# Tycro-Games/Raytracer-VoxPopuli

Measured on AMD Instinct MI355X. Metric: Mray/s (primary+shadow) at 1920×1080, 1024³ world; 1/2/4/8-GPU, higher is better.
Workload: dtype f32

## Files before the change

### raytracer-voxpopuli_amd/csrc/vpx_kernels.hip

```cpp
#include <hip/hip_runtime.h>
#include <hip/hip_gl_interop.h>
#include <rccl/rccl.h>

#include <algorithm>
#include <cmath>
#include <cstdio>
#include <cstdlib>
#include <cstring>
#include <string>
#include <array>
#include <atomic>
#include <vector>

#include "vpx_wavefront.hpp"
#include "vpx_model.hpp"
#include "vpx_noise.hpp"
#include "vpx_brush.hpp"

using namespace vpx;

namespace {

constexpr int kTile = 16;
#ifndef VPX_SPLIT_PRIMARY
// ... 1249 lines not shown
        free_fork(ws);
        return fail(c, VPX_E_DEVICE, "level fork: stream / event creation failed");
    }
    return VPX_OK;
}
void free_fork(vpx_ctx::WaveStore& ws) {
    if (ws.fork) (void)hipStreamSynchronize(ws.fork);
    if (ws.ev_fork) (void)hipEventDestroy(ws.ev_fork);
    if (ws.ev_join) (void)hipEventDestroy(ws.ev_join);
    if (ws.fork) (void)hipStreamDestroy(ws.fork);
    if (ws.fork_dedicated) g_lane_queues.fetch_sub(1);
    ws.fork = nullptr, ws.ev_fork = ws.ev_join = nullptr, ws.fork_dedicated = false;
}

static void prof_mark(vpx_ctx* c, hipStream_t s, int stage) {
    if (!c->prof_cap) return;
    if (stage >= 0 && !((c->prof_mask >> stage) & 1u)) return;
    if (stage >= 0 && c->prof_used + 2 > c->prof_cap) return;
    if (stage < 0 && (c->prof_used & 1u) == 0) return;
    if (hipEventRecord(c->prof_ev[c->prof_used], s) != hipSuccess) return;
    c->prof_stage[c->prof_used] = stage;
    ++c->prof_used;
}

struct Reproj {
    PrevCam prev;
    float4 *alb, *ill, *rd, *temp, *hist;
};

template <int MODE>
int launch_render(vpx_ctx* c, hipStream_t s, vpx_ctx::WaveStore& ws, const SceneView& sv, const FrameArgs& f,
                  uint32_t tiles, float4* accum, uint32_t* rgb8, float4* packed, const Reproj* rp = nullptr,
                  const hipEvent_t* tail_wait = nullptr, const WindowTail* wtail = nullptr) {
    const uint32_t P = tiles * (uint32_t)kTilePix;
    const uint32_t L = (uint32_t)std::max(1, f.max_bounces + 1);
    const uint32_t S = sv.num_areas ? (uint32_t)std::max(1, sv.area_samples) : 1u;
    int rc = ensure_wave(c, ws, P, L, S);
    if (rc) return rc;
    WaveBufs w = ws.w;
    if (rp) w.RD = rp->rd;
    const dim3 grid(tiles), block(kThreads);
    const size_t slds = sizeof(uint32_t) * S * kThreads;
    const bool one = sv.num_volumes == 1 && !(sv.num_spheres | sv.num_triangles);
    const bool x86 = sv.x86.tab != nullptr;
    const size_t xlds = x86 ? sizeof(uint32_t) * sv.x86.rsq_off : 0;
    const bool fuse_tail = !rp;
#ifndef VPX_SPOOL_ONE_SLOT
#define VPX_SPOOL_ONE_SLOT 1
#endif
#ifndef VPX_SPOOL_ONE_SERIAL
#define VPX_SPOOL_ONE_SERIAL 0
#endif
    const bool spool = !rp && (S > 1 || (one && VPX_SPOOL_ONE_SLOT && (VPX_SPOOL_ONE_SERIAL || &ws != &c->wave)));
    if (wtail && (!spool || f.max_bounces < 0 || !f.batch_tiles || tiles % wtail->B))
        return fail(c, VPX_E_INVALID, "window tail: needs a window chain with the shadow pool");
    if (!spool) w.occb = nullptr;
    const uint32_t sgrab = std::max(1u, std::min(4u, kShadowList / (64u * S)));
    auto resident = [&](uint32_t waves_per_simd) { return dim3(std::min(tiles, c->cus * waves_per_simd)); };
    auto shadow_pool = [&](int level) {
        const uint32_t grabs = (P / 64u + sgrab - 1u) / sgrab;
        const uint32_t waves = std::min(grabs, c->cus * 4u * (uint32_t)VPX_WPE_SPOOL);
        const uint32_t wpb = kPoolWg / 64u;
        hipLaunchKernelGGL(one ? k_shadow_pool<false> : k_shadow_pool<true>, dim3((waves + wpb - 1u) / wpb), dim3(kPoolWg), 0,
                           s, sv, w, level, sgrab, c->d_ctr);
        if (!one)
            hipLaunchKernelGGL(k_shadow_slots, dim3(std::min(tiles * S, c->cus * (uint32_t)VPX_WPE_SHADOW_SLOTS)), block, 0, s, sv,
                               w, level, c->d_ctr);
    };
    c->last_frame_kernel = 0;
    if (frame0_fits(sv, f, S, rp != nullptr) && tiles <= kFuseFrameTiles) {
        prof_mark(c, s, VPX_STAGE_FRAME);
#ifndef VPX_FRAME_EXTRA_LDS
#define VPX_FRAME_EXTRA_LDS 0
#endif
#ifndef VPX_FRAME_VIEWS
#define VPX_FRAME_VIEWS 2
#endif
        constexpr int kBase = VPX_FRAME_VIEWS >= 1 ? kFrameGuaranteed : kFrameAsGiven;
        constexpr int kLean = VPX_FRAME_VIEWS >= 2 ? kFrameLean : kBase;
        const bool lean = VPX_FRAME_VIEWS >= 2 && frame0_lean(sv, f);
        c->last_frame_kernel = lean ? 2 : 1;
        hipLaunchKernelGGL((lean ? (x86 ? k_frame0<true, MODE, true, kLean> : k_frame0<true, MODE, false, kLean>)
                                 : (x86 ? k_frame0<true, MODE, true, kBase> : k_frame0<true, MODE, false, kBase>)),
                           grid, block, slds + VPX_FRAME_EXTRA_LDS, s, sv, f, w, c->d_ctr, accum, rgb8, packed);
        prof_mark(c, s, -1);
        VPX_HIP(c, hipGetLastError());
        return VPX_OK;
    }
    VPX_HIP(c, hipMemsetAsync(w.pool, 0, sizeof(uint32_t) * kPoolWords, s));
    prof_mark(c, s, VPX_STAGE_PRIMARY);
    const bool fuse_head = f.max_bounces >= 0;
    const bool split = !one && fuse_head && VPX_SPLIT_PRIMARY && !(sv.num_spheres | sv.num_triangles);
    const bool defer = split && f.max_bounces == 0 && VPX_DEFER_INSTANCES;
    if (defer)
        hipLaunchKernelGGL((x86 ? k_primary<true, true, true, true> : k_primary<true, true, false, true>), grid, block, 0, s,
                           sv, f, w, c->d_ctr);
    else if (split)
        hipLaunchKernelGGL((x86 ? k_primary<true, false, true> : k_primary<true, false, false>), grid, block, 0, s, sv, f, w,
                           c->d_ctr);
    else if (fuse_head)
        hipLaunchKernelGGL((one ? (x86 ? k_primary<true, true, true> : k_primary<true, true, false>)
                                : (x86 ? k_primary<false, true, true> : k_primary<false, true, false>)),
                           grid, block, 0, s, sv, f, w,
                           c->d_ctr);
    else
        hipLaunchKernelGGL((one ? (x86 ? k_primary<true, false, true> : k_primary<true, false, false>)
                                : (x86 ? k_primary<false, false, true> : k_primary<false, false, false>)),
                           grid, block, 0, s, sv, f,
                           w, c->d_ctr);
    prof_mark(c, s, -1);
    if (split) {
        prof_mark(c, s, VPX_STAGE_INSTANCES);
        if (defer) {
            hipLaunchKernelGGL(k_compact, dim3((P / 64u + 255u) / 256u), block, 0, s, w, 0);
            hipLaunchKernelGGL(k_instances_list, grid, block, xlds, s, sv, f, w, c->d_ctr);
        } else {
            hipLaunchKernelGGL(k_instances, grid, block, xlds, s, sv, f, w, c->d_ctr);
        }
        prof_mark(c, s, -1);
    }
    auto bounce = [&](hipStream_t bs, int level) {
        prof_mark(c, bs, VPX_STAGE_BOUNCE);
        if (one) {
            const uint32_t chunks = (P + kPoolChunk - 1u) / kPoolChunk;
            const uint32_t waves = std::min(chunks, c->cus * 4u * (uint32_t)VPX_WPE_BOUNCE);
            const uint32_t wpb = kPoolWg / 64u;
            hipLaunchKernelGGL(x86 ? k_nearest_pool<true> : k_nearest_pool<false>, dim3((waves + wpb - 1u) / wpb),
                               dim3(kPoolWg), 0, bs, sv, w, level,
                               c->d_ctr);
        } else {
            hipLaunchKernelGGL(k_nearest_tile, grid, block, xlds, bs, sv, w, level, c->d_ctr);
        }
        prof_mark(c, bs, -1);
    };
    const bool fork = VPX_LEVEL_FORK && f.max_bounces > 0 && !rp && (&ws == &c->wave || (one && c->lanes.size() <= 2));
    if (fork && (rc = ensure_fork(c, ws))) return rc;
    const int tail_at = &ws == &c->wave ? VPX_TAIL_LEVEL - 1 : VPX_TAIL_LEVEL;
    const int tail_from = (VPX_TAIL_LEVEL > 0 && f.max_bounces >= VPX_TAIL_MIN_DEPTH && !rp) ? tail_at : -1;
    bool tailed = false;
    for (int level = 0; level <= f.max_bounces; ++level) {
        if (!(fuse_head && level == 0)) {
            prof_mark(c, s, VPX_STAGE_SHADE);
            hipLaunchKernelGGL(k_shade, grid, block, 0, s, sv, f, w, level, c->d_ctr);
            prof_mark(c, s, -1);
        }
        if (fuse_tail && level == f.max_bounces) {
            prof_mark(c, s, VPX_STAGE_SHADOW);
            if (spool)
                shadow_pool(level);
            else
                hipLaunchKernelGGL((one ? k_shadow_finish<true, MODE> : k_shadow_finish<false, MODE>), grid, block,
                                   slds, s, sv, f, w, c->d_ctr, accum, rgb8, packed);
            prof_mark(c, s, -1);
            if (spool) {
                if (tail_wait) VPX_HIP(c, hipStreamWaitEvent(s, *tail_wait, 0));
                prof_mark(c, s, VPX_STAGE_FINISH);
                if (wtail)
                    hipLaunchKernelGGL(k_finish_window<true>, dim3(tiles / wtail->B), block, 0, s, sv, f, w, *wtail,
                                       accum, rgb8);
                else
                    hipLaunchKernelGGL((k_resolve_finish<MODE>), grid, block, 0, s, sv, f, w, accum, rgb8, packed);
                prof_mark(c, s, -1);
            }
            break;
        }
        if (level < f.max_bounces)
            hipLaunchKernelGGL(k_compact, dim3((P / 64u + 255u) / 256u), block, 0, s, w, level);
// ... 1948 lines not shown
```

### raytracer-voxpopuli_amd/csrc/vpx_wavefront.hpp

```cpp
#pragma once

#include "vpx_trace.hpp"

namespace vpx {

constexpr int kTileW = 16;
constexpr int kTilePix = kTileW * kTileW;



constexpr uint32_t kActive = 1u;
constexpr uint32_t kInside = 2u;

constexpr uint32_t kSlotValid = 1u;
constexpr uint32_t kSlotDiscard = 2u;

constexpr uint32_t kFlagReproject = 0x80000000u;
constexpr uint32_t kPendZeroAdd = 1u << 13;

constexpr uint32_t kLightNone = 0, kLightSingle = 1, kLightArea = 2;

struct FrameArgs {
    vpx_camera cam;
    uint32_t width, height;
// ... 628 lines not shown
        base += i < wid ? v : 0u;
        total += v;
    }
    __syncthreads();
    return base + off;
}

template <class KIND = NearestWalk>
__device__ __forceinline__ void nearest_record(SceneView sv, const PathRay& pr, uint32_t p, Ray& r, Counters& k) {
    r.t = kBig;
    r.mat = kNone;
    r.N = mk(0.f, 0.f, 0.f);
    const int32_t vox = find_nearest<KIND>(sv, r, k);
    pr.H[pr.at(p)] = make_float4(r.t, r.N.x, r.N.y, r.N.z);
    pr.HM[pr.at(p)] = r.mat | ((uint32_t)(vox + 2) << 8) | (r.inside ? 0x80000000u : 0u);
}

__device__ __forceinline__ ORay path_oray(const vpx_volume& vol, const PathRay& pr, uint32_t p,
                                          const X86Arith& xa = X86Arith{}) {
    const float4 o = pr.O[pr.at(p)], d = pr.D[pr.at(p)];
    ORay r;
    r.O = xform_pos_ssem(mk(o.x, o.y, o.z), vol.inv_matrix);
    r.D = xform_vec_ssem(mk(d.x, d.y, d.z), vol.inv_matrix);
    r.rD = nearest_rd(r.D, xa);
    return r;
}

__device__ __forceinline__ bool nearest_begin_v(const vpx_volume& vol, uint32_t n, const PathRay& w, uint32_t p,
                                                Counters& k, skip::Walk& wk, const X86Arith& xa) {
    ++k.nearest;
    const ORay o = path_oray(vol, w, p, xa);
    Dda s;
    if (!dda_setup(vol, n, o, s)) return false;
    wk = to_walk(s);
    return true;
}
__device__ __forceinline__ bool nearest_begin_1v(const SceneView& sv, const PathRay& w, uint32_t p, Counters& k,
                                                 skip::Walk& wk) {
    const vpx_volume* vol = uni_ptr(&sv.volumes[0]);
    return nearest_begin_v(*vol, sv.grids[vol->grid_id].n, w, p, k, wk, sv.x86);
}
__device__ __forceinline__ void nearest_end_v(const vpx_volume& vol, const uint8_t* cells, uint32_t n, const PathRay& w,
                                              uint32_t p, const skip::Walk& wk, bool hit);
__device__ __forceinline__ void nearest_end_1v(const SceneView& sv, const PathRay& w, uint32_t p, const skip::Walk& wk,
                                               bool hit) {
    const vpx_volume* vol = uni_ptr(&sv.volumes[0]);
    const DevGrid g = sv.grids[vol->grid_id];
    nearest_end_v(*vol, g.cells, g.n, w, p, wk, hit);
}

template <class KIND = NearestWalk>
__device__ __forceinline__ void nearest_record_1v(const SceneView& sv, const PathRay& w, uint32_t p, Counters& k) {
    bool hit = false;
    skip::Walk wk;
    if (nearest_begin_1v(sv, w, p, k, wk))
        hit = walk_wave<KIND>(grid_view(sv.grids[uni_ptr(&sv.volumes[0])->grid_id]), wk, kBig, k.cells);
    nearest_end_1v(sv, w, p, wk, hit);
}

__device__ __forceinline__ void nearest_end_v(const vpx_volume& vol, const uint8_t* cells, uint32_t n, const PathRay& w,
                                              uint32_t p, const skip::Walk& wk, bool hit) {
    asm volatile("" ::: "memory");
    const uint32_t inside = __float_as_uint(w.D[w.at(p)].w) & kInside ? 0x80000000u : 0u;
    if (!hit) {
        w.H[w.at(p)] = make_float4(kBig, 0.f, 0.f, 0.f);
        w.HM[w.at(p)] = kNone | inside;
        return;
    }
    const ORay o = path_oray(vol, w, p);
    const f3 N = normal_voxel(o, wk.t, n, vol.matrix);
    const uint32_t mat = cells[(uint64_t)wk.X + (uint64_t)wk.Y * n + (uint64_t)wk.Z * ((uint64_t)n * n)];
    w.H[w.at(p)] = make_float4(wk.t, N.x, N.y, N.z);
    w.HM[w.at(p)] = mat | (2u << 8) | inside;
}

template <bool SHADE>
struct HeadLds {
    uint32_t sh[4];
    uint32_t lst[256];
    float4 ray[SHADE ? 3 * 256 : 1];
    uint32_t hm[SHADE ? 256 : 1];
};

__device__ __forceinline__ bool meets_later_volume(const SceneView& sv, f3 o, f3 d, float t) {
    if (!(sv.tlas_on && !sv.tlas_always && !(sv.num_spheres | sv.num_triangles) && sv.tlas_nodes)) return true;
    return tlas_box(sv.tlas[0], o, world_inv(d), t);
}

template <bool ONE, bool SHADE, class KIND = NearestWalk, bool DEFER = false>
__device__ __forceinline__ void primary_tile(const SceneView& sv, const FrameArgs& f, const WaveBufs& w,
                                             HeadLds<SHADE>& L, unsigned long long* __restrict__ ctr) {
    uint32_t* sh = L.sh;
    uint32_t* lst = L.lst;
    const uint32_t tb = tile_block() * 256u;
    const uint32_t p = tb + threadIdx.x;
    const PathRay pr = SHADE ? PathRay{L.ray, L.ray + 256, L.ray + 512, L.hm, tb} : PathRay{w.O, w.D, w.H, w.HM, 0u};
    Counters k{0u, 0u, 0u};
    uint32_t prim = 0;
    bool walk = false;
    if (p < w.P) {
        uint32_t x, y;
        bool go = path_pixel(f, p, x, y);
        if (!SHADE) {
            w.depth[p] = f.max_bounces;
            w.forms[p] = 1u;
        }
        Ray r;
        r.O = r.D = mk(0.f, 0.f, 0.f);
        uint32_t rng = 0, flags = 0;
        if (go) {
            Rng g{pixel_seed(f.seed_base, path_frame(f, p), f.width, f.height, x, y)};
            r = primary_ray(f, x, y, g, sv.x86);
            rng = g.s;
            prim = 1;
            flags = kActive;
        }
        if (f.max_bounces < 0) {
            go = false;
            flags = 0u;
        }
        pr.O[pr.at(p)] = make_float4(r.O.x, r.O.y, r.O.z, __uint_as_float(rng));
        pr.D[pr.at(p)] = make_float4(r.D.x, r.D.y, r.D.z, __uint_as_float(flags));
        if (SHADE && !flags && f.max_bounces > 0) w.D[p] = make_float4(0.f, 0.f, 0.f, __uint_as_float(0u));
        if (go) {
            walk = true;
            if (ONE) {
                const vpx_volume& vol = sv.volumes[0];
                ORay o;
                o.O = xform_pos_ssem(r.O, vol.inv_matrix);
                o.D = xform_vec_ssem(r.D, vol.inv_matrix);
                o.rD = nearest_rd(o.D, sv.x86);
                Dda s;
                if (!dda_setup(vol, sv.grids[vol.grid_id].n, o, s)) {
                    walk = false;
                    ++k.nearest;
                    pr.H[pr.at(p)] = make_float4(kBig, 0.f, 0.f, 0.f);
                    pr.HM[pr.at(p)] = kNone;
                }
            }
        }
    }
    uint32_t total;
    const uint32_t at = block_scan(walk ? 1u : 0u, total, sh);
    if (walk) lst[at] = p;
    __syncthreads();
    VPX_FRAME_PHASE(1);
    if (threadIdx.x < total) {
        const uint32_t q = lst[threadIdx.x];
        if (ONE) {
            nearest_record_1v<KIND>(sv, pr, q, k);
        } else {
            const float4 o = pr.O[pr.at(q)], d = pr.D[pr.at(q)];
            Ray r;
            r.O = mk(o.x, o.y, o.z);
            r.D = mk(d.x, d.y, d.z);
            r.inside = false;
            nearest_record(sv, pr, q, r, k);
        }
    }
    VPX_FRAME_PHASE(2);
    flush_counters(k, prim, ctr, VPX_STAGE_PRIMARY);
    if (SHADE) {
        __syncthreads();
        VPX_FRAME_PHASE(3);
        Counters ks{0u, 0u, 0u};
        bool defer = false;
        if (DEFER && p < w.P) {
            const float4 d = pr.D[pr.at(p)];
            if (__float_as_uint(d.w) & kActive) {
                const float4 o = pr.O[pr.at(p)], h = pr.H[pr.at(p)];
                defer = meets_later_volume(sv, mk(o.x, o.y, o.z), mk(d.x, d.y, d.z), h.x);
                if (defer) {
                    w.O[p] = o;
                    w.D[p] = d;
                    w.H[p] = h;
                    w.HM[p] = pr.HM[pr.at(p)];
                }
            }
        }
        if (DEFER) put_amask(w, p, defer);
        const bool cont = defer ? false : shade_path<true>(sv, f, w, pr, p, 0, ks);
        if (!DEFER && f.max_bounces > 0) put_amask(w, p, cont);
        flush_counters(ks, 0u, ctr, VPX_STAGE_SHADE);
    }
}

template <bool ONE, bool SHADE = false, bool X86 = false, bool DEFER = false>
__global__ __launch_bounds__(256) VPX_WPE(ONE ? VPX_WPE_NEAREST : VPX_WPE_MULTI_NEAREST) void k_primary(SceneView sv, FrameArgs f, WaveBufs w,
                                                 unsigned long long* __restrict__ ctr) {
    __shared__ HeadLds<SHADE> L;
    primary_tile<ONE, SHADE, NearestWalk, DEFER>(arith_view<X86>(sv), f, w, L, ctr);
}

__global__ __launch_bounds__(256) void k_compact(WaveBufs w, int level) {
    __shared__ uint32_t sh[4];
    __shared__ uint32_t base_s;
    const uint32_t n = live_count(w, level), words = (n + 63u) >> 6;
    if (blockIdx.x * 256u >= words) return;
    const uint32_t wi = blockIdx.x * 256u + threadIdx.x;
    uint64_t m = wi < words ? w.amask[wi] : 0ull;
    if (wi == words - 1u && (n & 63u)) m &= (1ull << (n & 63u)) - 1ull;
    uint32_t total;
    const uint32_t off = block_scan((uint32_t)__popcll(m), total, sh);
    if (threadIdx.x == 0) base_s = atomicAdd(&w.pool[kPoolLive + level + 1], total);
    __syncthreads();
    const uint32_t base = base_s;
    const uint32_t lane = threadIdx.x & 63u, w0 = blockIdx.x * 256u + (threadIdx.x & ~63u);
    const uint32_t* L = live_list(w, level);
    uint32_t* out = ((level + 1) & 1) ? w.live1 : w.live0;
    for (uint32_t j = 0; j < 64u; ++j) {
        const uint64_t mj = (uint64_t)(uint32_t)__builtin_amdgcn_readlane((int)(uint32_t)m, (int)j) |
                            (uint64_t)(uint32_t)__builtin_amdgcn_readlane((int)(uint32_t)(m >> 32), (int)j) << 32;
        if (!mj) continue;
        const uint32_t oj = (uint32_t)__builtin_amdgcn_readlane((int)off, (int)j);
        if ((mj >> lane) & 1ull) {
            const uint32_t i = (w0 + j) * 64u + lane;
            out[base + oj + lane_rank(mj)] = level ? L[i] : i;
        }
    }
}


__global__ __launch_bounds__(256) VPX_WPE(VPX_WPE_MULTI_NEAREST) void k_instances(SceneView sv_, FrameArgs f, WaveBufs w,
                                                                                unsigned long long* __restrict__ ctr) {
    __shared__ uint32_t sh[4];
    __shared__ uint32_t lst[256];
    extern __shared__ uint32_t x86_lds[];
    SceneView sv = sv_;
    sv.x86 = x86_stage_lds(sv_.x86, x86_lds);
    const uint32_t tb = tile_block() * 256u;
    const uint32_t p = tb + threadIdx.x;
    const PathRay pr{w.O, w.D, w.H, w.HM, 0u};
    Counters k{0u, 0u, 0u};
    bool go = false;
    if (p < w.P && (__float_as_uint(w.D[p].w) & kActive)) {
        const float4 o = w.O[p], d = w.D[p];
        go = meets_later_volume(sv, mk(o.x, o.y, o.z), mk(d.x, d.y, d.z), w.H[p].x);
    }
#ifdef VPX_DEBUG_NO_INST_WALK
    go = false;
#endif
    uint32_t total;
    const uint32_t at = block_scan(go ? 1u : 0u, total, sh);
    if (go) lst[at] = p;
    __syncthreads();
    if (threadIdx.x < total) {
        const uint32_t q = lst[threadIdx.x];
        const float4 o = w.O[q], d = w.D[q], h = w.H[q];
        const uint32_t hm = w.HM[q];
        Ray r;
        r.O = mk(o.x, o.y, o.z);
        r.D = mk(d.x, d.y, d.z);
        r.t = h.x;
        r.N = mk(h.y, h.z, h.w);
        r.mat = hm & 0xffu;
        r.inside = (hm & 0x80000000u) != 0u;
        int32_t vox = (int32_t)((hm >> 8) & 0xffffu) - 2;
        if (find_nearest_rest(sv, r, k, &vox)) {
            w.H[q] = make_float4(r.t, r.N.x, r.N.y, r.N.z);
            w.HM[q] = r.mat | ((uint32_t)(vox + 2) << 8) | (r.inside ? 0x80000000u : 0u);
        }
    }
    flush_counters(k, 0u, ctr, VPX_STAGE_INSTANCES);
    __syncthreads();
    Counters ks{0u, 0u, 0u};
// ... 55 lines not shown
            const uint32_t q = live_path(w, level + 1, i);
            const float4 o = w.O[q], d = w.D[q];
            Ray r;
            r.O = mk(o.x, o.y, o.z);
            r.D = mk(d.x, d.y, d.z);
            r.inside = (__float_as_uint(d.w) & kInside) != 0u;
            nearest_record<BounceWalk>(sv, PathRay{w.O, w.D, w.H, w.HM, 0u}, q, r, k);
        }
    }
    flush_counters(k, 0u, ctr, VPX_STAGE_BOUNCE);
}

#ifndef VPX_POOL_CHUNK
#define VPX_POOL_CHUNK 128
#endif
#ifndef VPX_POOL_LEAVE
#define VPX_POOL_LEAVE 16
#endif
#ifndef VPX_POOL_WG
#define VPX_POOL_WG 256
#endif
constexpr uint32_t kPoolChunk = VPX_POOL_CHUNK;
constexpr uint32_t kPoolLeave = VPX_POOL_LEAVE;
constexpr uint32_t kPoolWg = VPX_POOL_WG;
template <bool X86>
__global__ __launch_bounds__(kPoolWg) VPX_WPE(VPX_WPE_BOUNCE) void k_nearest_pool(SceneView sv_, WaveBufs w, int level,
                                                                               unsigned long long* __restrict__ ctr) {
    const SceneView sv = arith_view<X86>(sv_);
        const uint32_t n = live_count(w, level + 1);
    const uint32_t* L = live_list(w, level + 1);
    const PathRay pr{w.O, w.D, w.H, w.HM, 0u};
    const skip::GridView gv = grid_view(sv.grids[uni_ptr(&sv.volumes[0])->grid_id]);
    Counters k{0u, 0u, 0u};
    skip::Walk wk;
    uint32_t q = ~0u;
    int mode = kWalkMiss;
    uint32_t avail = 0u, cur = 0u;
    bool more = true;
    uint32_t line = pool_line0();
    for (;;) {
        if (q != ~0u && mode >= kWalkMiss) {
            nearest_end_1v(sv, pr, q, wk, mode == kWalkHit);
            q = ~0u;
        }
        while (more) {
            const uint64_t idle = __ballot(q == ~0u);
            if (!idle) break;
            if (avail == 0u) {
                const uint32_t g = pool_grab(w.pool + kPoolBounce + level * kGrabBlock, (n + kPoolChunk - 1u) / kPoolChunk, line);
                if (g == ~0u) {
                    more = false;
                    break;
                }
                cur = g * kPoolChunk;
                avail = min(kPoolChunk, n - cur);
                continue;
            }
            const uint32_t take = min((uint32_t)__popcll(idle), avail);
            const uint32_t r = lane_rank(idle);
            if (q == ~0u && r < take) {
                q = L[cur + r];
                mode = nearest_begin_1v(sv, pr, q, k, wk) ? kWalkStep : kWalkMiss;
            }
            cur += take;
            avail -= take;
        }
        if (!__ballot(q != ~0u)) break;
        walk_wave<BounceWalk, true>(gv, wk, kBig, k.cells, &mode,
                                                                   more ? kPoolLeave : 65u);
    }
    flush_counters(k, 0u, ctr, VPX_STAGE_BOUNCE);
}

constexpr uint32_t kOccWords = 15u * 256u / 32u;
__device__ __forceinline__ void mark_occluded(const WaveBufs& w, uint64_t slot, uint32_t e, uint32_t* occ) {
    if (occ) {
        const uint32_t b = (e >> 27) * 256u + (e & 255u);
        atomicOr(&occ[b >> 5], 1u << (b & 31u));
    } else {
        w.SD[slot].w = __uint_as_float(__float_as_uint(w.SD[slot].w) | 4u );
    }
}

template <bool ONE, class KIND = ShadowWalk>
__device__ __forceinline__ void shadow_tile(const SceneView& sv, const WaveBufs& w, unsigned long long* __restrict__ ctr,
                                            uint32_t* occ, uint32_t p, uint16_t* l16 = nullptr) {
    __shared__ uint32_t sh[4];
    if (occ)
        for (uint32_t i = threadIdx.x; i < w.S * 8u; i += 256u) occ[i] = 0u;
    extern __shared__ uint32_t lst_dyn[];
    Counters k{0u, 0u, 0u};
    __shared__ uint32_t hist[kLightKeys];
    if (threadIdx.x < kLightKeys) hist[threadIdx.x] = 0u;
    __syncthreads();
    const uint32_t sm = p < w.P ? w.smask[p] : 0u;
    const uint32_t m = sm & kSlotBits, key = sm >> 16;
    const uint32_t pos = m ? atomicAdd(&hist[key], (uint32_t)__popc(m)) : 0u;
    __syncthreads();
    uint32_t total = 0;
    if (threadIdx.x < 64) {
        const uint32_t v = threadIdx.x < kLightKeys ? hist[threadIdx.x] : 0u;
        uint32_t t;
        const uint32_t ex = wave_prefix(v, t);
        if (threadIdx.x < kLightKeys) hist[threadIdx.x] = ex;
        if (threadIdx.x == 0) sh[0] = t;
    }
    __syncthreads();
    total = __builtin_amdgcn_readfirstlane(sh[0]);
    const uint32_t tb = tile_block() * 256u;
    {
        uint32_t at = m ? hist[key] + pos : 0u;
        if (l16) {
            if (m) l16[at] = (uint16_t)(p - tb);
        } else {
            for (uint32_t b = m; b; b &= b - 1u) lst_dyn[at++] = ((uint32_t)__ffs(b) - 1u) << 27 | p;
        }
    }
    __syncthreads();
    VPX_FRAME_PHASE(5);
    for (uint32_t i = threadIdx.x; i < total; i += 256u) {
        const uint32_t e = l16 ? tb + l16[i] : lst_dyn[i];
        const uint64_t slot = (uint64_t)(e >> 27) * w.P + (e & 0x07ffffffu);
        if (ONE) {
            const vpx_volume* vol = uni_ptr(&sv.volumes[0]);
            const DevGrid g = sv.grids[vol->grid_id];
            ++k.shadow;
            bool hit = false;
            {
                const float4 so = w.SO[slot], sd = w.SD[slot];
                ORay o;
                o.O = xform_pos(mk(so.x, so.y, so.z), vol->inv_matrix);
                o.D = xform_vec(mk(sd.x, sd.y, sd.z), vol->inv_matrix);
                o.rD = mk(__fdiv_rn(1.0f, o.D.x), __fdiv_rn(1.0f, o.D.y), __fdiv_rn(1.0f, o.D.z));
                Dda s;
                if (dda_setup(*vol, g.n, o, s)) {
                    skip::Walk wk = to_walk(s);
                    hit = walk_wave<KIND>(grid_view(g), wk, so.w, k.cells);
                }
            }
            asm volatile("" ::: "memory");
            if (hit) mark_occluded(w, slot, e, occ);
            continue;
        }
        const float4 so = w.SO[slot], sd = w.SD[slot];
        Ray r;
        r.O = mk(so.x, so.y, so.z);
        r.D = mk(sd.x, sd.y, sd.z);
        r.t = so.w;
        if (shadow(sv, r, k)) mark_occluded(w, slot, e, occ);
    }
    VPX_FRAME_PHASE(6);
    flush_counters(k, 0u, ctr, VPX_STAGE_SHADOW);
}

template <bool ONE>
__global__ __launch_bounds__(256) VPX_WPE(ONE ? VPX_WPE_SHADOW : VPX_WPE_MULTI_SHADOW) void k_shadow_tile(SceneView sv, WaveBufs w, unsigned long long* __restrict__ ctr) {
    shadow_tile<ONE>(sv, w, ctr, nullptr, tile_block() * 256u + threadIdx.x);
}

template <bool ONE>
__global__ __launch_bounds__(256) VPX_WPE(ONE ? VPX_WPE_SHADOW : VPX_WPE_MULTI_SHADOW) void k_shadow_list(SceneView sv, WaveBufs w, int level,
                                                                                                       unsigned long long* __restrict__ ctr) {
    const uint32_t n = live_count(w, level);
    if (blockIdx.x * 256u >= n) return;
    const uint32_t i = blockIdx.x * 256u + threadIdx.x;
    shadow_tile<ONE>(sv, w, ctr, nullptr, i < n ? live_path(w, level, i) : ~0u);
}

constexpr uint32_t kShadowList = 1024;
#ifndef VPX_WPE_SPOOL
#define VPX_WPE_SPOOL 5
#endif
template <bool MULTI>
__global__ __launch_bounds__(kPoolWg) VPX_WPE(VPX_WPE_SPOOL) void k_shadow_pool(SceneView sv, WaveBufs w, int level,
                                                                              uint32_t grab,
                                                                              unsigned long long* __restrict__ ctr) {
    __shared__ uint32_t lst_wg[kPoolWg / 64][kShadowList];
    __shared__ uint32_t hist_wg[kPoolWg / 64][kLightKeys];
    uint32_t* lst = lst_wg[__builtin_amdgcn_readfirstlane(threadIdx.x >> 6)];
    uint32_t* hist = hist_wg[__builtin_amdgcn_readfirstlane(threadIdx.x >> 6)];
    const uint32_t lane = threadIdx.x & 63u;
    const uint32_t n = live_count(w, level);
    const uint32_t grabs = (n + 64u * grab - 1u) / (64u * grab);
    const vpx_volume* vol = uni_ptr(&sv.volumes[0]);
    const DevGrid g = sv.grids[vol->grid_id];
    const skip::GridView gv = grid_view(g);
    Counters k{0u, 0u, 0u};
    skip::Walk wk;
    uint32_t e = ~0u;
    uint32_t walked = 0u;
    float bound = 0.f;
    int mode = kWalkMiss;
    uint32_t avail = 0u, cur = 0u;
    bool more = true;
    uint32_t line = pool_line0();
    for (;;) {
        if constexpr (!MULTI) {
            if (e != ~0u && mode >= kWalkMiss) {
                w.occb[(uint64_t)(e >> 27) * w.P + (e & 0x07ffffffu)] = mode == kWalkHit ? 1u : 0u;
                e = ~0u;
            }
        } else {
            const bool fin = e != ~0u && mode >= kWalkMiss;
            bool app = false;
// ... 314 lines not shown
        return;
    }
    float4 a = accum[at];
    const uint32_t stride = f.batch_tiles * 256u;
    for (uint32_t b = 0; b < wt.B; ++b) {
        const uint32_t p = p0 + b * stride;
        f3 v;
        if (RESOLVE) {
            LightSum ls;
            resolve_path(sv, w, p, nullptr, &ls);
            v = path_value(w, p, &ls);
        } else {
            v = path_value(w, p, nullptr);
        }
        a = blend(a, v, wt.ww.w[b], wt.ww.iw[b]);
    }
    accum[at] = a;
    if (rgb8) rgb8[at] = tonemap_pack(a);
}

#ifndef VPX_WPE_TAIL
#define VPX_WPE_TAIL 2
#endif
__global__ __launch_bounds__(256) VPX_WPE(VPX_WPE_TAIL) void k_tail(SceneView sv_, FrameArgs f, WaveBufs w, int level,
                                                      unsigned long long* __restrict__ ctr) {
    Counters kn{0u, 0u, 0u}, ks{0u, 0u, 0u}, kh{0u, 0u, 0u};
    const uint32_t n = live_count(w, level);
    const uint32_t i = blockIdx.x * 256u + threadIdx.x;
    if (blockIdx.x * 256u >= n) return;
    extern __shared__ uint32_t x86_lds[];
    SceneView sv = sv_;
    sv.x86 = x86_stage_lds(sv_.x86, x86_lds);
    const uint32_t p = i < n ? live_path(w, level, i) : ~0u;
    const PathRay pr{w.O, w.D, w.H, w.HM, 0u};
    for (int l = level; p != ~0u; ++l) {
        {
            const float4 o = w.O[p], d = w.D[p];
            Ray r;
            r.O = mk(o.x, o.y, o.z);
            r.D = mk(d.x, d.y, d.z);
            r.inside = (__float_as_uint(d.w) & kInside) != 0u;
            nearest_record<BounceWalk>(sv, pr, p, r, kn);
        }
        const bool cont = shade_path(sv, f, w, pr, p, l, kh);
        const uint32_t slots = w.smask[p] & kSlotBits;
        for (uint32_t b = slots; b; b &= b - 1u) {
            const uint64_t slot = (uint64_t)((uint32_t)__ffs(b) - 1u) * w.P + p;
            const float4 so = w.SO[slot], sd = w.SD[slot];
            Ray r;
            r.O = mk(so.x, so.y, so.z);
            r.D = mk(sd.x, sd.y, sd.z);
            r.t = so.w;
            if (shadow(sv, r, ks)) w.SD[slot].w = __uint_as_float(__float_as_uint(sd.w) | 4u );
        }
        resolve_path(sv, w, p);
        if (!cont || l >= f.max_bounces) break;
    }
    flush_counters(kn, 0u, ctr, VPX_STAGE_BOUNCE);
    flush_counters(ks, 0u, ctr, VPX_STAGE_SHADOW);
    flush_counters(kh, 0u, ctr, VPX_STAGE_SHADE);
}

template <bool ONE, int MODE>
__global__ __launch_bounds__(256) VPX_WPE(ONE ? VPX_WPE_SHADOW : VPX_WPE_MULTI_SHADOW) void k_shadow_finish(
    SceneView sv, FrameArgs f, WaveBufs w, unsigned long long* __restrict__ ctr, float4* __restrict__ accum,
    uint32_t* __restrict__ rgb8, float4* __restrict__ packed) {
    __shared__ uint32_t occ[kOccWords];
    shadow_tile<ONE>(sv, w, ctr, occ, tile_block() * 256u + threadIdx.x);
    __syncthreads();
    uint32_t p = tile_block() * 256u + threadIdx.x;
    asm volatile("" : "+v"(p));
    LightSum ls;
    resolve_path(sv, w, p, occ, &ls);
    finish_path<MODE>(f, w, p, accum, rgb8, packed, &ls);
}

#ifndef VPX_FUSE_FRAME_TILES
#define VPX_FUSE_FRAME_TILES 12288
#endif
constexpr uint32_t kFuseFrameTiles = VPX_FUSE_FRAME_TILES;
#ifndef VPX_WPE_FRAME
#define VPX_WPE_FRAME 7
#endif
enum : int { kFrameAsGiven = 0, kFrameGuaranteed = 1, kFrameLean = 2 };

inline bool frame0_fits(const SceneView& sv, const FrameArgs& f, uint32_t slots, bool reproject) {
    return sv.num_volumes == 1 && !(sv.num_spheres | sv.num_triangles) && f.max_bounces == 0 && !reproject &&
           !(f.flags & kFlagReproject) && slots == 1 && !f.batch_tiles;
}
inline bool frame0_lean(const SceneView& sv, const FrameArgs& f) {
    return !sv.num_spots && !sv.num_areas && !sv.sky_tex && !(f.flags & (VPX_FLAG_DOF | VPX_FLAG_SKY));
}
template <bool X86, int VIEW>
__device__ __forceinline__ SceneView frame0_scene(const SceneView& sv) {
    SceneView v = arith_view<X86>(sv);
    if (VIEW >= kFrameGuaranteed) {
        v.num_volumes = 1;
        v.num_spheres = v.num_triangles = 0;
        v.tlas_on = 0;
    }
    if (VIEW >= kFrameLean) {
        v.num_spots = v.num_areas = 0;
        v.area_samples = 1;
        v.sky_tex = 0;
    }
    return v;
}
template <int VIEW>
__device__ __forceinline__ FrameArgs frame0_args(const FrameArgs& f) {
    FrameArgs v = f;
    v.batch_tiles = 0;
    if (VIEW >= kFrameGuaranteed) {
        v.max_bounces = 0;
        v.flags &= ~kFlagReproject;
    }
    if (VIEW >= kFrameLean) v.flags &= ~(uint32_t)(VPX_FLAG_DOF | VPX_FLAG_SKY);
    return v;
}

template <bool ONE, int MODE, bool X86 = false, int VIEW = kFrameAsGiven>
__global__ __launch_bounds__(256) VPX_WPE(ONE ? VPX_WPE_FRAME : VPX_WPE_MULTI_NEAREST) void k_frame0(
    SceneView sv_, FrameArgs f_, WaveBufs w, unsigned long long* __restrict__ ctr, float4* __restrict__ accum,
    uint32_t* __restrict__ rgb8, float4* __restrict__ packed) {
    VPX_FRAME_PHASE(0);
    const SceneView sv = frame0_scene<X86, VIEW>(sv_);
    const FrameArgs f = frame0_args<VIEW>(f_);
    __shared__ HeadLds<true> L;
    __shared__ float4 s_val[256];
    __shared__ float4 s_sm[256];
    __shared__ uint32_t occ[8];
    __shared__ uint16_t l16[256];
    const uint32_t tb = tile_block() * 256u;
    const uint32_t p = tb + threadIdx.x;
    WaveBufs wl = w;
    wl.LA = s_val - tb;
    wl.leaf = s_val - tb;
    wl.SM = s_sm - tb;
    wl.smask = L.hm - tb;
    wl.forms = L.lst - tb;
    wl.SO = L.ray - tb;
    wl.SD = L.ray + 256 - tb;
    wl.SL = L.ray + 512 - tb;
    if (VIEW >= kFrameGuaranteed) wl.S = 1u;
    primary_tile<ONE, true, FrameNearestWalk>(sv, f, wl, L, ctr);
    __syncthreads();
    VPX_FRAME_PHASE(4);
#ifdef VPX_FRAME_P_TILE
    shadow_tile<ONE, FrameShadowWalk>(sv, wl, ctr, occ, tile_block() * 256u + threadIdx.x, l16);
#else
    uint32_t ps = p;
    asm volatile("" : "+v"(ps));
    shadow_tile<ONE, FrameShadowWalk>(sv, wl, ctr, occ, ps, l16);
#endif
    __syncthreads();
    VPX_FRAME_PHASE(7);
    uint32_t pt = p;
    asm volatile("" : "+v"(pt));
    LightSum ls;
    resolve_path(sv, wl, pt, occ, &ls);
    finish_path<MODE>(f, wl, pt, accum, rgb8, packed, &ls);
    VPX_FRAME_PHASE(8);
}


struct PrevCam {
    f3 pos, left, right, top, bottom;
};

__global__ __launch_bounds__(256) void k_finish_reproject(FrameArgs f, WaveBufs w, float4* __restrict__ alb,
                                                          float4* __restrict__ ill) {
    const uint32_t p = blockIdx.x * 256u + threadIdx.x;
    if (p >= w.P) return;
    uint32_t x, y;
    if (!path_pixel_single(f, p, x, y)) return;
    const uint64_t px = (uint64_t)y * f.width + x;
    f3 A = mk(0.f, 0.f, 0.f), I = mk(0.f, 0.f, 0.f);
    if (f.max_bounces < 0) {
        const float4 o = w.O[p], d = w.D[p];
        const f3 ip = mk(o.x, o.y, o.z) + mk(d.x, d.y, d.z) * kBig;
        w.RD[px] = make_float4(ip.x, ip.y, ip.z, __uint_as_float(kNone));
    } else {
        const uint32_t forms = w.forms[p];
        f3 v = mk(0.f, 0.f, 0.f);
        if (forms & kLeafBit) {
            const float4 lf = w.leaf[p];
            v = mk(lf.x, lf.y, lf.z);
        }
        const int nl = (int)forms_count(forms);
        if (nl == 0) {
            A = v;
            I = mk(1.f, 1.f, 1.f);
        } else {
            for (int i = nl - 1; i >= 1; --i) {
                const uint32_t form = (forms >> (2 * i)) & 3u;
                const uint64_t li = (uint64_t)i * w.P + p;
                const float4 a4 = w.LA[li];
                const f3 a = mk(a4.x, a4.y, a4.z);
                if (form == kFormAddMul) {
                    const float4 b4 = w.LB[li];
                    v = (v + mk(b4.x, b4.y, b4.z)) * a;
                } else {
                    v = v * a;
                }
            }
            const float4 a4 = w.LA[p];
            A = mk(a4.x, a4.y, a4.z);
            if ((forms & 3u) == kFormAddMul) {
                const float4 b4 = w.LB[p];
                I = v + mk(b4.x, b4.y, b4.z);
            } else {
                I = v;
            }
        }
    }
    alb[px] = make_float4(A.x, A.y, A.z, 0.f);
    ill[px] = make_float4(I.x, I.y, I.z, 0.f);
}

__global__ __launch_bounds__(256) void k_reproject_setup(FrameArgs f, WaveBufs w, PrevCam pc) {
    const uint32_t p = blockIdx.x * 256u + threadIdx.x;
    if (p >= w.P) return;
    uint32_t x, y;
    uint32_t slots = 0;
    w.SM[p] = make_float4(0.f, 0.f, 0.f, __uint_as_float(0u));
    if (path_pixel_single(f, p, x, y)) {
        const float4 rd = w.RD[(uint64_t)y * f.width + x];
        const f3 P = mk(rd.x, rd.y, rd.z);
        const f3 delta = P - pc.pos;
        const float ld = dot(pc.left, delta), rdist = dot(pc.right, delta);
        const float td = dot(pc.top, delta), bd = dot(pc.bottom, delta);
        const float u = ld / (ld + rdist), v = td / (td + bd);
        const float hw = (1.0f / (float)f.width) / 2.0f, hh = (1.0f / (float)f.height) / 2.0f;
        const float uu = u + hw, vv = v + hh;
        const bool valid = uu >= 0.0f && uu < 1.0f && vv >= 0.0f && vv < 1.0f;
        w.SM[p] = make_float4(uu, vv, 0.f, __uint_as_float(valid ? 1u : 0u));
// ... 101 lines not shown
```

Before: 6884.

## Stash primary DDA setup in LDS to skip recomputation in fused frame kernel

Result: faster. 7001, median of 6 (+1.7%).

```diff
diff --git a/raytracer-voxpopuli_amd/csrc/vpx_kernels.hip b/raytracer-voxpopuli_amd/csrc/vpx_kernels.hip
--- a/raytracer-voxpopuli_amd/csrc/vpx_kernels.hip
+++ b/raytracer-voxpopuli_amd/csrc/vpx_kernels.hip
@@ -1355,7 +1355,7 @@
         c->last_frame_kernel = lean ? 2 : 1;
         hipLaunchKernelGGL((lean ? (x86 ? k_frame0<true, MODE, true, kLean> : k_frame0<true, MODE, false, kLean>)
                                  : (x86 ? k_frame0<true, MODE, true, kBase> : k_frame0<true, MODE, false, kBase>)),
-                           grid, block, slds + VPX_FRAME_EXTRA_LDS, s, sv, f, w, c->d_ctr, accum, rgb8, packed);
+                           grid, block, VPX_FRAME_EXTRA_LDS, s, sv, f, w, c->d_ctr, accum, rgb8, packed);
         prof_mark(c, s, -1);
         VPX_HIP(c, hipGetLastError());
         return VPX_OK;
diff --git a/raytracer-voxpopuli_amd/csrc/vpx_wavefront.hpp b/raytracer-voxpopuli_amd/csrc/vpx_wavefront.hpp
--- a/raytracer-voxpopuli_amd/csrc/vpx_wavefront.hpp
+++ b/raytracer-voxpopuli_amd/csrc/vpx_wavefront.hpp
@@ -734,14 +734,48 @@
     uint32_t hm[SHADE ? 256 : 1];
 };
 
+struct WalkStash {
+    float4 *a, *b, *c;
+};
+__device__ __forceinline__ void stash_put(const WalkStash& st, uint32_t i, const Dda& s) {
+    const uint32_t sg = (s.sx < 0 ? 1u : 0u) | (s.sy < 0 ? 2u : 0u) | (s.sz < 0 ? 4u : 0u);
+    st.a[i] = make_float4(__uint_as_float(s.X), __uint_as_float(s.Y), __uint_as_float(s.Z), __uint_as_float(sg));
+    st.b[i] = make_float4(s.t, s.tmax.x, s.tmax.y, s.tmax.z);
+    st.c[i] = make_float4(s.tdelta.x, s.tdelta.y, s.tdelta.z, 0.f);
+}
+__device__ __forceinline__ skip::Walk stash_get(const WalkStash& st, uint32_t i) {
+    const float4 a = st.a[i], b = st.b[i], c = st.c[i];
+    const uint32_t sg = __float_as_uint(a.w);
+    skip::Walk w;
+    w.X = __float_as_uint(a.x), w.Y = __float_as_uint(a.y), w.Z = __float_as_uint(a.z);
+    w.t = b.x;
+    w.tx = b.y, w.ty = b.z, w.tz = b.w;
+    w.dx = c.x, w.dy = c.y, w.dz = c.z;
+    w.sx = sg & 1u ? -1 : 1, w.sy = sg & 2u ? -1 : 1, w.sz = sg & 4u ? -1 : 1;
+    skip::walk_begin(w);
+    return w;
+}
+template <class KIND>
+__device__ __forceinline__ void nearest_record_stashed(const SceneView& sv, const PathRay& w, const uint32_t* lst,
+                                                       Counters& k, const WalkStash& st) {
+    ++k.nearest;
+    skip::Walk wk = stash_get(st, w.at(lst[threadIdx.x]));
+    const bool hit = walk_wave<KIND>(grid_view(sv.grids[uni_ptr(&sv.volumes[0])->grid_id]), wk, kBig, k.cells);
+    uint32_t i = threadIdx.x;
+    asm volatile("" : "+v"(i) : : "memory");
+    nearest_end_1v(sv, w, lst[i], wk, hit);
+}
+
 __device__ __forceinline__ bool meets_later_volume(const SceneView& sv, f3 o, f3 d, float t) {
     if (!(sv.tlas_on && !sv.tlas_always && !(sv.num_spheres | sv.num_triangles) && sv.tlas_nodes)) return true;
     return tlas_box(sv.tlas[0], o, world_inv(d), t);
 }
 
-template <bool ONE, bool SHADE, class KIND = NearestWalk, bool DEFER = false>
+template <bool ONE, bool SHADE, class KIND = NearestWalk, bool DEFER = false, bool STASH = false>
 __device__ __forceinline__ void primary_tile(const SceneView& sv, const FrameArgs& f, const WaveBufs& w,
-                                             HeadLds<SHADE>& L, unsigned long long* __restrict__ ctr) {
+                                             HeadLds<SHADE>& L, unsigned long long* __restrict__ ctr,
+                                             const WalkStash* st = nullptr) {
+    static_assert(!STASH || (ONE && SHADE), "the walk stash is the fused single-volume head's");
     uint32_t* sh = L.sh;
     uint32_t* lst = L.lst;
     const uint32_t tb = tile_block() * 256u;
@@ -788,9 +822,17 @@
                     ++k.nearest;
                     pr.H[pr.at(p)] = make_float4(kBig, 0.f, 0.f, 0.f);
                     pr.HM[pr.at(p)] = kNone;
+                } else if (STASH) {
+                    stash_put(*st, pr.at(p), s);
                 }
             }
         }
+    }
+    uint32_t carried = 0u;
+    if (STASH) {
+        carried = prim | k.nearest << 1;
+        asm volatile("" : "+v"(carried));
+        prim = k.nearest = 0u;
     }
     uint32_t total;
     const uint32_t at = block_scan(walk ? 1u : 0u, total, sh);
@@ -799,7 +841,9 @@
     VPX_FRAME_PHASE(1);
     if (threadIdx.x < total) {
         const uint32_t q = lst[threadIdx.x];
-        if (ONE) {
+        if (ONE && STASH) {
+            nearest_record_stashed<KIND>(sv, pr, lst, k, *st);
+        } else if (ONE) {
             nearest_record_1v<KIND>(sv, pr, q, k);
         } else {
             const float4 o = pr.O[pr.at(q)], d = pr.D[pr.at(q)];
@@ -811,28 +855,35 @@
         }
     }
     VPX_FRAME_PHASE(2);
+    uint32_t ps = p;
+    if (STASH) {
+        prim = carried & 1u;
+        k.nearest += carried >> 1;
+        ps = tb + threadIdx.x;
+        asm volatile("" : "+v"(ps));
+    }
     flush_counters(k, prim, ctr, VPX_STAGE_PRIMARY);
     if (SHADE) {
         __syncthreads();
         VPX_FRAME_PHASE(3);
         Counters ks{0u, 0u, 0u};
         bool defer = false;
-        if (DEFER && p < w.P) {
-            const float4 d = pr.D[pr.at(p)];
+        if (DEFER && ps < w.P) {
+            const float4 d = pr.D[pr.at(ps)];
             if (__float_as_uint(d.w) & kActive) {
-                const float4 o = pr.O[pr.at(p)], h = pr.H[pr.at(p)];
+                const float4 o = pr.O[pr.at(ps)], h = pr.H[pr.at(ps)];
                 defer = meets_later_volume(sv, mk(o.x, o.y, o.z), mk(d.x, d.y, d.z), h.x);
                 if (defer) {
-                    w.O[p] = o;
-                    w.D[p] = d;
-                    w.H[p] = h;
-                    w.HM[p] = pr.HM[pr.at(p)];
+                    w.O[ps] = o;
+                    w.D[ps] = d;
+                    w.H[ps] = h;
+                    w.HM[ps] = pr.HM[pr.at(ps)];
                 }
             }
         }
-        if (DEFER) put_amask(w, p, defer);
-        const bool cont = defer ? false : shade_path<true>(sv, f, w, pr, p, 0, ks);
-        if (!DEFER && f.max_bounces > 0) put_amask(w, p, cont);
+        if (DEFER) put_amask(w, ps, defer);
+        const bool cont = defer ? false : shade_path<true>(sv, f, w, pr, ps, 0, ks);
+        if (!DEFER && f.max_bounces > 0) put_amask(w, ps, cont);
         flush_counters(ks, 0u, ctr, VPX_STAGE_SHADE);
     }
 }
@@ -1054,9 +1105,10 @@
     }
 }
 
+constexpr uint32_t kShadowTileLds = sizeof(uint32_t) * (4u + kLightKeys);
 template <bool ONE, class KIND = ShadowWalk>
 __device__ __forceinline__ void shadow_tile(const SceneView& sv, const WaveBufs& w, unsigned long long* __restrict__ ctr,
-                                            uint32_t* occ, uint32_t p, uint16_t* l16 = nullptr) {
+                                            uint32_t* occ, uint32_t p, float4* lw = nullptr) {
     __shared__ uint32_t sh[4];
     if (occ)
         for (uint32_t i = threadIdx.x; i < w.S * 8u; i += 256u) occ[i] = 0u;
@@ -1082,8 +1134,8 @@
     const uint32_t tb = tile_block() * 256u;
     {
         uint32_t at = m ? hist[key] + pos : 0u;
-        if (l16) {
-            if (m) l16[at] = (uint16_t)(p - tb);
+        if (lw) {
+            if (m) lw[at].w = __uint_as_float(p - tb);
         } else {
             for (uint32_t b = m; b; b &= b - 1u) lst_dyn[at++] = ((uint32_t)__ffs(b) - 1u) << 27 | p;
         }
@@ -1091,7 +1143,7 @@
     __syncthreads();
     VPX_FRAME_PHASE(5);
     for (uint32_t i = threadIdx.x; i < total; i += 256u) {
-        const uint32_t e = l16 ? tb + l16[i] : lst_dyn[i];
+        const uint32_t e = lw ? tb + __float_as_uint(lw[i].w) : lst_dyn[i];
         const uint64_t slot = (uint64_t)(e >> 27) * w.P + (e & 0x07ffffffu);
         if (ONE) {
             const vpx_volume* vol = uni_ptr(&sv.volumes[0]);
@@ -1572,6 +1624,9 @@
 #ifndef VPX_WPE_FRAME
 #define VPX_WPE_FRAME 7
 #endif
+#ifndef VPX_FRAME_HANDOFF
+#define VPX_FRAME_HANDOFF 1
+#endif
 enum : int { kFrameAsGiven = 0, kFrameGuaranteed = 1, kFrameLean = 2 };
 
 inline bool frame0_fits(const SceneView& sv, const FrameArgs& f, uint32_t slots, bool reproject) {
@@ -1608,6 +1663,16 @@
     return v;
 }
 
+struct Frame0Lds {
+    HeadLds<true> L;
+    float4 s_val[256];
+    float4 s_sm[256];
+    uint32_t occ[8];
+};
+constexpr uint32_t kFrame0LdsBudget = 23040;
+static_assert(sizeof(Frame0Lds) + kShadowTileLds <= kFrame0LdsBudget,
+              "k_frame0: seven workgroups no longer fit a CU's LDS (22576 + 80 = 22656 today)");
+
 template <bool ONE, int MODE, bool X86 = false, int VIEW = kFrameAsGiven>
 __global__ __launch_bounds__(256) VPX_WPE(ONE ? VPX_WPE_FRAME : VPX_WPE_MULTI_NEAREST) void k_frame0(
     SceneView sv_, FrameArgs f_, WaveBufs w, unsigned long long* __restrict__ ctr, float4* __restrict__ accum,
@@ -1615,11 +1680,11 @@
     VPX_FRAME_PHASE(0);
     const SceneView sv = frame0_scene<X86, VIEW>(sv_);
     const FrameArgs f = frame0_args<VIEW>(f_);
-    __shared__ HeadLds<true> L;
-    __shared__ float4 s_val[256];
-    __shared__ float4 s_sm[256];
-    __shared__ uint32_t occ[8];
-    __shared__ uint16_t l16[256];
+    __shared__ Frame0Lds F;
+    HeadLds<true>& L = F.L;
+    float4* const s_val = F.s_val;
+    float4* const s_sm = F.s_sm;
+    uint32_t* const occ = F.occ;
     const uint32_t tb = tile_block() * 256u;
     const uint32_t p = tb + threadIdx.x;
     WaveBufs wl = w;
@@ -1632,15 +1697,18 @@
     wl.SD = L.ray + 256 - tb;
     wl.SL = L.ray + 512 - tb;
     if (VIEW >= kFrameGuaranteed) wl.S = 1u;
-    primary_tile<ONE, true, FrameNearestWalk>(sv, f, wl, L, ctr);
+    constexpr bool kStash = ONE && VPX_FRAME_HANDOFF;
+    const WalkStash st{L.ray + 512, s_val, s_sm};
+    primary_tile<ONE, true, FrameNearestWalk, false, kStash>(sv, f, wl, L, ctr, &st);
     __syncthreads();
     VPX_FRAME_PHASE(4);
+    float4* const lw = L.ray + 512;
 #ifdef VPX_FRAME_P_TILE
-    shadow_tile<ONE, FrameShadowWalk>(sv, wl, ctr, occ, tile_block() * 256u + threadIdx.x, l16);
+    shadow_tile<ONE, FrameShadowWalk>(sv, wl, ctr, occ, tile_block() * 256u + threadIdx.x, lw);
 #else
     uint32_t ps = p;
     asm volatile("" : "+v"(ps));
-    shadow_tile<ONE, FrameShadowWalk>(sv, wl, ctr, occ, ps, l16);
+    shadow_tile<ONE, FrameShadowWalk>(sv, wl, ctr, occ, ps, lw);
 #endif
     __syncthreads();
     VPX_FRAME_PHASE(7);
```
